# jianwang-mpi/GlobalEgoMocap

Hardware: AMD Instinct MI355X
Metric: optimised windows/sec (10-frame, 15-joint) (higher is better)
Workload: dtype f32

## Files before the change

globalegomocap_amd/csrc/energy.hip:

```cpp
#include "energy_device.h"

namespace gem {

__global__ void pack_pose_kernel(const float* __restrict__ src, float* __restrict__ dst, int rows, int C) {
    const int i = blockIdx.x * blockDim.x + threadIdx.x;
    if (i >= rows * PAD) return;
    const int r = i / PAD, c = i % PAD;
    dst[i] = c < C ? src[(size_t)r * C + c] : 0.f;
}
__global__ void unpack_pose_kernel(const float* __restrict__ src, float* __restrict__ dst, int rows, int C) {
    const int i = blockIdx.x * blockDim.x + threadIdx.x;
    if (i >= rows * C) return;
    const int r = i / C, c = i % C;
    dst[i] = src[(size_t)r * PAD + c];
}
int launch_pack_pose(const float* src, float* dst, int rows, int C, hipStream_t s) {
    const int n = rows * PAD;
    hipLaunchKernelGGL(pack_pose_kernel, dim3((n + 255) / 256), dim3(256), 0, s, src, dst, rows, C);
    GEM_HIP(hipGetLastError());
    return 0;
}
int launch_unpack_pose(const float* src, float* dst, int rows, int C, hipStream_t s) {
    const int n = rows * C;
    hipLaunchKernelGGL(unpack_pose_kernel, dim3((n + 255) / 256), dim3(256), 0, s, src, dst, rows, C);
// ... 78 lines not shown
    hipLaunchKernelGGL(energy_kernel, dim3(B), dim3(64), 0, s, a);
    GEM_HIP(hipGetLastError());
    if (prof) { GEM_HIP(hipEventRecord(rec.b, s)); h->prof.recs.push_back(rec); }
    commit_kernel_names(h, prof ? rec.family : -1);
    return 0;
}

__global__ __launch_bounds__(256) void mean_bone_kernel(const float* __restrict__ pose, int n_frames, int J,
                                                        const int* __restrict__ parents, float* __restrict__ out) {
    __shared__ float red[4][MAXJ];
    const int tid = threadIdx.x, lane = tid & 63, wave = tid >> 6;
    for (int j = 0; j < J; ++j) {
        float acc = 0.f;
        const int par = parents[j];
        for (int f = tid; f < n_frames; f += 256) {
            const float* a = pose + ((size_t)f * J + j) * 3;
            const float* p = pose + ((size_t)f * J + par) * 3;
            const float dx = a[0] - p[0], dy = a[1] - p[1], dz = a[2] - p[2];
            acc += sqrtf(dx * dx + dy * dy + dz * dz);
        }
#pragma unroll
        for (int o = 32; o > 0; o >>= 1) acc += __shfl_xor(acc, o, 64);
        if (lane == 0) red[wave][j] = acc;
    }
    __syncthreads();
    if (tid < J) out[tid] = (red[0][tid] + red[1][tid] + red[2][tid] + red[3][tid]) / (float)n_frames;
}
int launch_mean_bone(gem_handle* h, const float* pose, int n_frames, float* out, hipStream_t s) {
    hipLaunchKernelGGL(mean_bone_kernel, dim3(1), dim3(256), 0, s, pose, n_frames, h->J, h->d_parents, out);
    GEM_HIP(hipGetLastError());
    return 0;
}

__global__ void gather_windows_kernel(const float* __restrict__ frames, const int32_t* __restrict__ frame0,
                                      float* __restrict__ out, int B, int T, int JC) {
    const int i = blockIdx.x * blockDim.x + threadIdx.x;
    if (i >= B * T * JC) return;
    const int b = i / (T * JC), r = i - b * T * JC;
    out[i] = frames[(size_t)frame0[b] * JC + r];
}
int launch_gather_windows(const float* frames, const int32_t* frame0, float* out, int B, int T, int JC, hipStream_t s) {
    const int n = B * T * JC;
    hipLaunchKernelGGL(gather_windows_kernel, dim3((n + 255) / 256), dim3(256), 0, s, frames, frame0, out, B, T, JC);
    GEM_HIP(hipGetLastError());
    return 0;
}

__device__ void inv4_rigid_general(const double* m, double* o) {
    const double a = m[0], b = m[1], c = m[2], d = m[4], e = m[5], f = m[6], g = m[8], hh = m[9], i = m[10];
    const double A = e * i - f * hh, Bc = -(d * i - f * g), Cc = d * hh - e * g;
    const double det = a * A + b * Bc + c * Cc;
    const double id = 1.0 / det;
    double r[9] = {A * id, -(b * i - c * hh) * id, (b * f - c * e) * id,
                   Bc * id, (a * i - c * g) * id, -(a * f - c * d) * id,
                   Cc * id, -(a * hh - b * g) * id, (a * e - b * d) * id};
    const double tx = m[3], ty = m[7], tz = m[11];
    for (int q = 0; q < 3; ++q) {
        o[q * 4 + 0] = r[q * 3 + 0]; o[q * 4 + 1] = r[q * 3 + 1]; o[q * 4 + 2] = r[q * 3 + 2];
        o[q * 4 + 3] = -(r[q * 3 + 0] * tx + r[q * 3 + 1] * ty + r[q * 3 + 2] * tz);
    }
    o[12] = 0; o[13] = 0; o[14] = 0; o[15] = 1;
}

__global__ __launch_bounds__(64) void relative_global_kernel(const float* __restrict__ local, const double* __restrict__ cams,
                                                             const int32_t* __restrict__ frame0, float* __restrict__ rel,
                                                             int T, int J) {
    __shared__ double M[MAXT][12];
    const int b = blockIdx.x, lane = threadIdx.x;
    const double* c0 = cams + (size_t)frame0[b] * 16;
    if (lane < T) {
        double inv0[16];
        inv4_rigid_general(c0, inv0);
        const double* ct = c0 + (size_t)lane * 16;
        for (int r = 0; r < 3; ++r)
            for (int c = 0; c < 4; ++c) {
                double acc = 0;
                for (int k = 0; k < 4; ++k) acc += inv0[r * 4 + k] * ct[k * 4 + c];
                M[lane][r * 4 + c] = acc;
            }
    }
    __syncthreads();
    for (int p = lane; p < T * J; p += 64) {
        const int t = p / J;
        const float* x = local + ((size_t)b * T * J + p) * 3;
        const double X = x[0], Y = x[1], Z = x[2];
        float* o = rel + ((size_t)b * T * J + p) * 3;
        for (int r = 0; r < 3; ++r)
            o[r] = (float)(M[t][r * 4 + 0] * X + M[t][r * 4 + 1] * Y + M[t][r * 4 + 2] * Z + M[t][r * 4 + 3]);
    }
}
__global__ __launch_bounds__(64) void to_global_kernel(const float* __restrict__ rel, const double* __restrict__ cams,
                                                       const int32_t* __restrict__ frame0, double* __restrict__ out, int T, int J) {
    const int b = blockIdx.x, lane = threadIdx.x;
    const double* c0 = cams + (size_t)frame0[b] * 16;
    for (int p = lane; p < T * J; p += 64) {
        const float* x = rel + ((size_t)b * T * J + p) * 3;
        const double X = x[0], Y = x[1], Z = x[2];
        double* o = out + ((size_t)b * T * J + p) * 3;
        for (int r = 0; r < 3; ++r) o[r] = c0[r * 4 + 0] * X + c0[r * 4 + 1] * Y + c0[r * 4 + 2] * Z + c0[r * 4 + 3];
    }
}
int launch_relative_global(const float* local, const double* cams, const int32_t* frame0, float* rel, int B, int T, int J,
                           hipStream_t s) {
    hipLaunchKernelGGL(relative_global_kernel, dim3(B), dim3(64), 0, s, local, cams, frame0, rel, T, J);
    GEM_HIP(hipGetLastError());
    return 0;
}
int launch_to_global(const float* rel, const double* cams, const int32_t* frame0, double* out, int B, int T, int J,
                     hipStream_t s) {
    hipLaunchKernelGGL(to_global_kernel, dim3(B), dim3(64), 0, s, rel, cams, frame0, out, T, J);
    GEM_HIP(hipGetLastError());
    return 0;
}

}
```

globalegomocap_amd/csrc/gem_api.hip:

```cpp
#include <cxxabi.h>

#include <algorithm>
#include <cmath>
#include <cstdio>
#include <cstdlib>
#include <cstring>
#include <memory>

#include "gem_internal.h"

namespace gem {

static thread_local std::string g_error;
void set_error(const std::string& msg) { g_error = msg; }
bool hip_ok(hipError_t e, const char* what) {
    if (e == hipSuccess) return true;
    g_error = std::string(what) + ": " + hipGetErrorString(e);
    return false;
}

const char* dev_env(const char* name) {
    const char* on = getenv("GEM_DEV");
    if (!on || on[0] != '1') return nullptr;
    return getenv(name);
}

void note_kernel(gem_handle* h, const void* host_fn) {
    if (!h->prof.on) return;
    const char* m = hipKernelNameRefByPtr(host_fn, nullptr);
    if (!m) return;
    int st = 0;
    char* d = abi::__cxa_demangle(m, nullptr, nullptr, &st);
    std::string n = (st == 0 && d) ? d : m;
    free(d);
    if (n.rfind("void ", 0) == 0) n = n.substr(5);
    int depth = 0;
    for (size_t i = 0; i < n.size(); ++i) {
        if (n[i] == '<') ++depth;
        else if (n[i] == '>') --depth;
        else if (n[i] == '(' && depth == 0) { n.resize(i); break; }
    }
    h->prof.pending.insert(n);
}

static void drop_graphs(gem_handle* h) {
    for (auto& g : h->graphs) { if (g.exec) (void)hipGraphExecDestroy(g.exec); if (g.graph) (void)hipGraphDestroy(g.graph); }
    h->graphs.clear();
}

__global__ void fill_u32_kernel(uint32_t* __restrict__ p, uint32_t v, size_t n) {
    const size_t i = (size_t)blockIdx.x * blockDim.x + threadIdx.x;
    if (i < n) p[i] = v;
}
static int launch_fill_u32(uint32_t* p, uint32_t v, size_t n, hipStream_t s) {
    if (!n) return 0;
    hipLaunchKernelGGL(fill_u32_kernel, dim3((unsigned)((n + 255) / 256)), dim3(256), 0, s, p, v, n);
    GEM_HIP(hipGetLastError());
    return 0;
}

template <typename T>
static int dev_alloc(std::vector<void*>& owner, T** p, size_t n) {
    void* q = nullptr;
    GEM_HIP(hipMalloc(&q, (n ? n : 1) * sizeof(T)));
    owner.push_back(q);
    *p = static_cast<T*>(q);
    GEM_HIP(hipMemset(q, 0, (n ? n : 1) * sizeof(T)));
    return 0;
}
static void free_all(std::vector<void*>& owner) {
    for (void* p : owner) (void)hipFree(p);
    owner.clear();
}

template <typename T>
static int upload(std::vector<void*>& owner, T** p, const std::vector<T>& v) {
    if (dev_alloc(owner, p, v.size())) return 1;
    GEM_HIP(hipMemcpy(*p, v.data(), v.size() * sizeof(T), hipMemcpyHostToDevice));
    return 0;
}

static uint16_t host_f2bf(float x) {
    uint32_t u;
    std::memcpy(&u, &x, 4);
    return (uint16_t)((u + 0x7FFFu + ((u >> 16) & 1u)) >> 16);
}
static float host_bf2f(uint16_t b) {
    const uint32_t u = (uint32_t)b << 16;
    float f;
    std::memcpy(&f, &u, 4);
    return f;
// ... 331 lines not shown
        net.dec_bwd.push_back(Lb);
        return 0;
    };
    for (int i = nh - 1; i >= 1; --i)
        if (add_dec(c.hidden[i], c.hidden[i - 1], true, true)) return 1;
    if (add_dec(c.hidden[0], c.hidden[0], true, true)) return 1;
    if (add_dec(c.hidden[0], C, false, false)) return 1;
    net.tail_start = -1;
    if (!dev_env("GEM_NO_TAIL"))
        for (int st = 1; st < (int)net.dec.size(); ++st) {
            const size_t bytes = plan_tail(net.dec, st, T, h->J, nullptr);
            if (bytes && bytes <= 160 * 1024) { net.tail_start = st; net.tail_lds = bytes; break; }
        }
    if (net.tail_start == 1 && !dev_env("GEM_NO_FRONT") && compose_front(h, net, first_conv, dec_in_bias_tm.data())) return 1;
    if (build_tail_bf16_stream(h, net)) return 1;
    net.host_fwd.clear(); net.host_fwd.shrink_to_fit();
    net.host_bwd.clear(); net.host_bwd.shrink_to_fit();
    net.loaded = true;
    return 0;
}

}

namespace gem {

static int check_call(gem_handle* h, int stage, int B, const char* who) {
    if (!h) { set_error(std::string(who) + ": null handle"); return 1; }
    if (stage < 0 || stage > 1 || !h->net[stage].loaded) { set_error(std::string(who) + ": VAE weights of this stage are not loaded"); return 1; }
    if (B < 0 || B > h->ws.Bmax) { set_error(std::string(who) + ": B exceeds max_windows"); return 1; }
    GEM_HIP(hipSetDevice(h->cfg.device));
    return 0;
}

static int encoder_forward(gem_handle* h, int stage, int B, const float* d_pose, hipStream_t s) {
    StageNet& net = h->net[stage];
    Workspace& w = h->ws;
    const int rows = B * h->T;
    if (launch_pack_pose(d_pose, w.pose_p, rows, h->C, s)) return 1;
    const float* in = w.pose_p;
    int lda = PAD;
    for (size_t i = 0; i < net.enc.size(); ++i) {
        if (launch_gemm(h, net.enc[i], EPI_BIAS_LRELU, in, lda, nullptr, w.enc_act[i], net.enc[i].N, rows, h->T, s, -1)) return 1;
        in = w.enc_act[i];
        lda = net.enc[i].N;
    }
    return launch_gemm(h, net.fc, EPI_BIAS, in, net.fc.K, nullptr, w.mulv, net.fc.N, B, h->T, s, -1);
}

static int decoder_forward(gem_handle* h, int stage, int B, const float* zp, hipStream_t s) {
    StageNet& net = h->net[stage];
    Workspace& w = h->ws;
    const int rows = B * h->T;
    const bool front = net.front.w && net.dec.size() > 1 && h->precision != GEM_PRECISION_BF16;
    const float* in = w.h0;
    if (front) {
        if (launch_gemm(h, net.front, EPI_BIAS_LRELU, zp, h->Dp, nullptr, w.dec_act[0], net.front.N, B, h->T, s, 0, w.dyn ? w.perm : nullptr)) return 1;
        in = w.dec_act[0];
    } else if (launch_gemm(h, net.dec_in, EPI_BIAS, zp, h->Dp, nullptr, w.h0, net.dec_in.N, B, h->T, s, 0, w.dyn ? w.perm : nullptr)) {
        return 1;
    }
    for (size_t i = front ? 1 : 0; i < net.dec.size(); ++i) {
        const int epi = (i + 1 < net.dec.size()) ? EPI_BIAS_LRELU : EPI_BIAS;
        if (launch_gemm(h, net.dec[i], epi, in, net.dec[i].K, nullptr, w.dec_act[i], net.dec[i].N, rows, h->T, s, -1)) return 1;
        in = w.dec_act[i];
    }
    return 0;
}

static int decoder_backward(gem_handle* h, int stage, int B, hipStream_t s, int from, const float* gin) {
    StageNet& net = h->net[stage];
    Workspace& w = h->ws;
// ... 74 lines not shown
    ta.B = B; ta.forward_only = forward_only ? 1 : 0; ta.dbg_ts = nullptr;
    ta.in_slab = in_slab; ta.in_bias = front ? net.front.bias : net.dec[st - 1].bias;
    ta.in_bias_ld = front ? net.dec[0].N : 0;
    for (int i = 0; i < ta.n; ++i) {
        const Layer& f = net.dec[st + i];
        const Layer& g = net.dec_bwd[st + i];
        ta.fwd[i] = TailLayerDev{f.w4, f.bias, f.K, f.N};
        ta.bwd[i] = TailLayerDev{g.w4, nullptr, g.K, g.N};
    }
    ta.a_in = w.dec_act[st - 1]; ta.g_out = w.dec_grad[st]; ta.g_out_b = nullptr; ta.Xp = (w.dyn && !forward_only) ? nullptr : w.dec_act.back();
    ta.e = ea;
    if (launch_tail(h, ta, tail_lds, s)) return 1;
    if (forward_only) return 0;
    if (front) {
        w.defer_reduce = w.dyn;
        const int rc = launch_gemm(h, net.front_bwd, EPI_BIAS, w.dec_grad[st], net.front_bwd.K, nullptr, w.dz, h->Dp, B, h->T, s, 0);
        w.grad_slab = w.defer_reduce ? w.deferred : SlabSrc{};
        w.defer_reduce = false;
        return rc;
    }
    return decoder_backward(h, stage, B, s, st - 1, w.dec_grad[st]);
}

struct StageRun {
    gem_handle* h = nullptr;
    int stage = 0, B = 0;
    const float* pose_in = nullptr; const float* heat = nullptr; const int32_t* frame0 = nullptr; const float* mean_bone = nullptr;
    const float* eps = nullptr;
    gem_energy_weights wt{}; gem_lbfgs_opts opt{};
    float* pose_out = nullptr; gem_window_stats* stats = nullptr;
    hipStream_t s = nullptr;
    EnergyArgs ea{};
    bool fuse = false;
    bool atomic_slots = false;
    long log0 = 0;
    int rounds = 0;
};

static void compaction_home(Workspace& w) {
    w.perm = w.perm_home; w.slot_of = w.slot_of_home; w.n_active = w.n_active_home;
    w.next_perm = w.next_slot_of = w.next_count = nullptr;
}

static int stage_begin(StageRun& r) {
    gem_handle* h = r.h;
    Workspace& w = h->ws;
    const int B = r.B, stage = r.stage;
    hipStream_t s = r.s;
    if (r.wt.reproj != 0.0 && (!r.heat || !r.frame0)) { set_error("optimize: reproj weight != 0 needs heat-maps and frame indices"); return 1; }
    if (r.opt.max_iter < 1 || r.opt.max_eval < 1 || r.opt.max_iter - 1 > w.hist_cap || r.opt.max_iter > MAX_HIST) {
        set_error("optimize: max_iter must be 1.." + std::to_string(w.hist_cap + 1)); return 1;
    }
    if (r.opt.max_eval > 1021) { set_error("optimize: max_eval must be at most 1021 (torch's default for max_iter = 25 is 31)"); return 1; }
    r.rounds = r.opt.max_eval + 1;
    if (B == 0) return 0;
    if (encoder_forward(h, stage, B, r.pose_in, s)) return 1;
    if (launch_reparam(w.mulv, r.eps, nullptr, nullptr, nullptr, w.trial, B, h->D, h->Dp, s)) return 1;
    if (h->precision == GEM_PRECISION_BF16 && launch_f32_to_bf16(w.trial, w.trial_b, (size_t)B * h->Dp, s)) return 1;
    if (launch_lbfgs_init(h, B, r.opt, s)) return 1;
    compaction_home(w);
    StageNet& net_ = h->net[stage];
    const bool front_ = net_.front.w && net_.tail_start == 1 && h->precision != GEM_PRECISION_BF16;
    const Layer& first_ = front_ ? net_.front : net_.dec_in;
    const int tail_g_ = h->T <= 16 ? 16 / h->T : 1;
    const bool tail_path_ = net_.tail_start >= 0 && (B + tail_g_ - 1) / tail_g_ <= tail_cap_workgroups(h, net_.dec, net_.tail_start);
    const bool fuse_ = tail_path_ && rows_can_fuse_compaction(h, first_, h->Dp, first_.N, B, front_);
    r.atomic_slots = bf16_rounds_take_slots_atomically(h, stage, B) ||
                     (h->precision == GEM_PRECISION_F32 && front_ && tail_path_ && !fuse_);
    if (r.atomic_slots) {
        if ((w.log_pos % N_LOG) + r.rounds + 2 > N_LOG) w.log_pos += N_LOG - (w.log_pos % N_LOG);
        r.log0 = w.log_pos;
    }
    if (launch_compact(h, B, 1, s, r.atomic_slots ? r.rounds + 1 : 0)) return 1;
    if (r.atomic_slots) w.log_pos = r.log0 + r.rounds + 2;
    w.dyn = true;
    w.tex_on = h->tex_cache && w.tex_key && r.wt.reproj != 0.0;
    if (w.tex_on && launch_fill_u32(reinterpret_cast<uint32_t*>(w.tex_key), 0xFFFFFFFFu, (size_t)B * h->T * h->J, s)) return 1;
    r.ea = energy_args(h, r.pose_in, r.heat, r.frame0, r.mean_bone, r.wt);
    w.tex_on = false;
    if (launch_fill_u32(reinterpret_cast<uint32_t*>(w.trace), 0xFFFFFFFFu, (size_t)TRACE_ROUNDS * w.Bmax * 2, s)) return 1;
    r.fuse = fuse_;
    return 0;
}

static int stage_round(StageRun& r, int k) {
    gem_handle* h = r.h;
    Workspace& w = h->ws;
    if (r.B == 0) return 0;
    int rc = 0;
    w.round = k;
    if (r.atomic_slots) {
        int* cnt = w.n_log + (r.log0 + k) % N_LOG;
        w.perm = (k & 1) ? w.perm2 : w.perm_home;       w.next_perm = (k & 1) ? w.perm_home : w.perm2;
        w.slot_of = (k & 1) ? w.slot_of2 : w.slot_of_home; w.next_slot_of = (k & 1) ? w.slot_of_home : w.slot_of2;
        w.n_active = cnt; w.next_count = cnt + 1;
        w.cur_log = r.log0 + k;
        r.ea.n_dev = w.n_active; r.ea.perm = w.perm;
    } else
    if (k > 0) {
        if (r.fuse) {
            w.fuse_compact = true;
            w.fuse_log = w.n_log + (w.log_pos % N_LOG);
            w.cur_log = w.log_pos++;
        } else {
            rc = launch_compact(h, r.B, 0, r.s);
        }
    }
    rc = rc || evaluate(h, r.stage, r.B, w.trial, r.ea, r.s);
    if (!rc) rc = launch_lbfgs_advance(h, r.B, r.opt, r.s);
    if (w.fuse_compact) { set_error("optimize: the fused compaction was not picked up"); rc = 1; w.fuse_compact = false; }
    w.round = -1;
    return rc;
}

static int stage_finish(StageRun& r) {
    gem_handle* h = r.h;
    Workspace& w = h->ws;
    w.round = -1;
    w.dyn = false;
    compaction_home(w);
    if (r.B == 0) return 0;
    if (evaluate(h, r.stage, r.B, w.trial, energy_args(h, r.pose_in, r.heat, r.frame0, r.mean_bone, r.wt), r.s, true)) return 1;
    if (launch_unpack_pose(w.dec_act.back(), r.pose_out, r.B * h->T, h->C, r.s)) return 1;
    if (r.stats && launch_lbfgs_stats(h, r.B, r.stats, r.s)) return 1;
    return 0;
}

static int optimize_stage_impl(gem_handle* h, int stage, int B, const float* d_pose_in, const float* d_heat,
                               const int32_t* d_frame0, const float* d_mean_bone, const float* d_eps,
                               const gem_energy_weights& wt, const gem_lbfgs_opts& opt, float* d_pose_out,
                               gem_window_stats* d_stats, hipStream_t s) {
    StageRun r;
    r.h = h; r.stage = stage; r.B = B; r.pose_in = d_pose_in; r.heat = d_heat; r.frame0 = d_frame0; r.mean_bone = d_mean_bone; r.eps = d_eps;
    r.wt = wt; r.opt = opt; r.pose_out = d_pose_out; r.stats = d_stats; r.s = s;
    if (stage_begin(r)) { h->ws.dyn = false; compaction_home(h->ws); return 1; }
    int rc = 0;
    for (int k = 0; k < r.rounds && !rc; ++k) rc = stage_round(r, k);
    if (rc) { h->ws.round = -1; h->ws.dyn = false; compaction_home(h->ws); return 1; }
    return stage_finish(r);
}

struct WindowsRun {
    gem_handle* h = nullptr;
    int B = 0;
    const float* local_pose = nullptr; const double* cams = nullptr; const float* heat = nullptr; const int32_t* frame0 = nullptr;
    const float* mean_bone = nullptr; const float* eps_local = nullptr; const float* eps_global = nullptr;
    gem_energy_weights w_local{}, w_global{}; gem_lbfgs_opts opt{};
    float* mid_local = nullptr; double* global = nullptr; gem_window_stats* stats_local = nullptr; gem_window_stats* stats_global = nullptr;
    hipStream_t s = nullptr;
    StageRun st;
    float* mid = nullptr;
};

static int windows_begin_local(WindowsRun& r) {
    gem_handle* h = r.h;
    Workspace& w = h->ws;
    if (launch_gather_windows(r.local_pose, r.frame0, w.pose_a, r.B, h->T, h->C, r.s)) return 1;
    r.mid = r.mid_local ? r.mid_local : w.pose_b;
    StageRun& s = r.st;
    s = StageRun{};
    s.h = h; s.stage = GEM_STAGE_LOCAL; s.B = r.B; s.pose_in = w.pose_a; s.heat = r.heat; s.frame0 = r.frame0; s.mean_bone = r.mean_bone;
    s.eps = r.eps_local; s.wt = r.w_local; s.opt = r.opt; s.pose_out = r.mid; s.stats = r.stats_local; s.s = r.s;
    return stage_begin(s);
}
static int windows_begin_global(WindowsRun& r) {
    gem_handle* h = r.h;
    Workspace& w = h->ws;
    if (stage_finish(r.st)) return 1;
    if (launch_relative_global(r.mid, r.cams, r.frame0, w.pose_a, r.B, h->T, h->J, r.s)) return 1;
    StageRun& s = r.st;
    s = StageRun{};
    s.h = h; s.stage = GEM_STAGE_GLOBAL; s.B = r.B; s.pose_in = w.pose_a; s.heat = r.heat; s.frame0 = r.frame0; s.mean_bone = r.mean_bone;
    s.eps = r.eps_global; s.wt = r.w_global; s.opt = r.opt; s.pose_out = w.pose_b;
    s.stats = r.stats_global; s.s = r.s;
    return stage_begin(s);
}
static int windows_end(WindowsRun& r) {
    gem_handle* h = r.h;
    if (stage_finish(r.st)) return 1;
    return launch_to_global(h->ws.pose_b, r.cams, r.frame0, r.global, r.B, h->T, h->J, r.s);
}
static void windows_abort(WindowsRun& r) { r.h->ws.round = -1; r.h->ws.dyn = false; compaction_home(r.h->ws); }

static int windows_single(WindowsRun& r) {
    int rc = windows_begin_local(r);
    for (int k = 0; k < r.st.rounds && !rc; ++k) rc = stage_round(r.st, k);
    rc = rc || windows_begin_global(r);
    for (int k = 0; k < r.st.rounds && !rc; ++k) rc = stage_round(r.st, k);
    rc = rc || windows_end(r);
    if (rc) windows_abort(r);
    return rc;
}

static bool same_key(const GraphKey& a, const GraphKey& b) {
    if (a.kind != b.kind || a.stage != b.stage || a.B != b.B || a.precision != b.precision || a.stream != b.stream || a.tex_cache != b.tex_cache)
        return false;
    for (int i = 0; i < 12; ++i)
        if (a.ptr[i] != b.ptr[i]) return false;
    return std::memcmp(a.w, b.w, sizeof(a.w)) == 0 && std::memcmp(&a.opt, &b.opt, sizeof(a.opt)) == 0;
}

template <typename Body>
static int run_graphed(gem_handle* h, const GraphKey& key, hipStream_t s, Body body) {
    if (!h->graphs_on || s == nullptr || h->prof.on) return body();
    GraphEntry* e = nullptr;
    for (auto& g : h->graphs)
        if (same_key(g.key, key)) { e = &g; break; }
    ++h->graph_tick;
    if (!e) {
        if (h->graphs.size() >= 16) {
            size_t lru = 0;
            for (size_t i = 1; i < h->graphs.size(); ++i)
                if (h->graphs[i].last_use < h->graphs[lru].last_use) lru = i;
// ... 294 lines not shown
```

globalegomocap_amd/csrc/gem_internal.h:

```cpp
#pragma once
#if defined(__HIP_DEVICE_COMPILE__) && !defined(GEM_NO_PACKED_FP32)
#error "compile with: -Xclang -target-feature -Xclang -packed-fp32-ops -DGEM_NO_PACKED_FP32 (__graft_entry__.NO_PACKED_FP32)"
#endif

#include <hip/hip_runtime.h>
#include <stdint.h>
#include <atomic>
#include <set>
#include <string>
#include <vector>

#include "../../include/gem_hip.h"

namespace gem {

constexpr int PAD = 64;
constexpr float LEAKY_SLOPE = 0.01f;
constexpr double BN_EPS = 1e-5;
constexpr int MAX_HIST = 128;
constexpr int MAXJ_ERR = GEM_MAX_JOINTS;
constexpr int N_LOG = 1 << 16;
constexpr int TRACE_ROUNDS = 64;

inline int pad64(int x) { return (x + PAD - 1) / PAD * PAD; }
// ... 181 lines not shown
    int64_t graph_replays = 0, graph_captures = 0;
    int* d_parents = nullptr;
    int* d_children = nullptr;
};

namespace gem {

void note_kernel(gem_handle* h, const void* host_fn);
inline void commit_kernel_names(gem_handle* h, int family) {
    if (family >= 0 && family < 4) h->prof.names[family].insert(h->prof.pending.begin(), h->prof.pending.end());
    h->prof.pending.clear();
}

int launch_gemm(gem_handle* h, const Layer& L, int epi, const float* A, int lda, const float* aux, float* Cout, int ldc,
                int M, int T, hipStream_t s, int family, const int* row_map = nullptr);

int pick_splitk(const gem_handle* h, long blocks, int n_tiles, size_t slab_elems);

struct DynSplit { int RT, SK, per; size_t slab; };
__host__ __device__ inline DynSplit dyn_split(int M, int BM, int CT, int W, int n_tiles, int ldc) {
    DynSplit d;
    d.RT = (M + BM - 1) / BM;
    if (d.RT < 1) d.RT = 1;
    int cap = W / (d.RT * CT);
    if (cap < 1) cap = 1;
    int mx = n_tiles / 4;
    if (mx < 1) mx = 1;
    const int sk = cap < mx ? cap : mx;
    d.per = (n_tiles + sk - 1) / sk;
    d.SK = (n_tiles + d.per - 1) / d.per;
    d.slab = (size_t)d.RT * BM * ldc;
    return d;
}
__device__ inline void slab_layout(const SlabSrc& s, int& nslab, size_t& stride) {
    nslab = s.nslab;
    stride = s.stride;
    if (s.dyn_W > 0) {
        const DynSplit d = dyn_split(*s.m_dev, 64, s.CT, s.dyn_W, s.n_tiles, s.ldc);
        nslab = d.SK;
        stride = d.slab;
    }
}
bool rows_can_fuse_compaction(const gem_handle* h, const Layer& L, int lda, int ldc, int B, bool slabs);
bool bf16_rounds_take_slots_atomically(const gem_handle* h, int stage, int B);
int launch_splitk_reduce(gem_handle* h, int epi, int nslab, size_t slab, const float* bias, const float* aux, float* C, int M, int N,
                         int ldc, const int* m_dev, hipStream_t s, int dyn_W = 0, int n_tiles = 0);
int launch_gemm_bf16(gem_handle* h, const Layer& L, int epi, int nprod, const float* A, int lda, const float* aux, float* Cout,
                     int ldc, int M, int T, hipStream_t s, const int* row_map);

struct EnergyArgs;
int evaluate_bf16(gem_handle* h, int stage, int B, const EnergyArgs& ea, hipStream_t s, bool forward_only);
int launch_f32_to_bf16(const float* src, uint16_t* dst, size_t n, hipStream_t s);
int launch_f32_split_bf16(const float* src, uint16_t* hi, uint16_t* lo, size_t n, hipStream_t s);

int launch_pack_pose(const float* src, float* dst, int rows, int C, hipStream_t s);
int launch_unpack_pose(const float* src, float* dst, int rows, int C, hipStream_t s);
int launch_reparam(const float* mulv, const float* eps, float* mu, float* logvar, float* z, float* z2, int B, int D, int Dp,
                   hipStream_t s);
int launch_pad_latent(const float* z, float* zp, int B, int D, int Dp, hipStream_t s);
int launch_unpad_latent(const float* zp, float* z, int B, int D, int Dp, hipStream_t s);

struct EnergyArgs {
    const float* Xp;
    const float* X0;
    const float* heat;
    const int32_t* frame0;
// ... 33 lines not shown
    int off_act[TAIL_MAX_LAYERS + 1], ld_act[TAIL_MAX_LAYERS + 1], off_g[2], ld_g, off_red, off_escr, off_zero, off_pre;
    EnergyArgs e;
};
size_t plan_tail(const std::vector<Layer>& dec, int start, int T, int J, TailArgs* out, bool shared = false);
size_t plan_tail_for(const gem_handle* h, const std::vector<Layer>& dec, int start, int wgs, TailArgs* out);

constexpr int TB_MAX_LAYERS = 6;
struct TailB16Layer { int K, N; const float* bias; };
struct TailB16Args {
    int n, B, G, nrt, forward_only, mask_first;
    SlabSrc in_slab;
    const float* in_bias;
    int in_bias_ld;
    const uint16_t* a_in_b;
    uint16_t* g_out_b;
    float* Xp;
    long long* dbg_ts;
    const uint16_t* wstream;
    int steps_f, steps_total;
    TailB16Layer fwd[TB_MAX_LAYERS], bwd[TB_MAX_LAYERS];
    int off_act[TB_MAX_LAYERS + 1], ld_act[TB_MAX_LAYERS + 1];
    int off_mask[TB_MAX_LAYERS], ld_mask[TB_MAX_LAYERS];
    int off_x, escr, off_mb, off_zero, off_tab;
    int off_bwin, off_epair;
    EnergyArgs e;
};
size_t plan_tail_bf16(const std::vector<Layer>& dec, int start, int T, int J, TailB16Args* out, int nrt = 5);
int tail_bf16_row_tiles(const gem_handle* h, int B, int T);
int build_tail_bf16_stream(gem_handle* h, StageNet& net);
int launch_tail_bf16(gem_handle* h, const TailB16Args& a, size_t lds_bytes, hipStream_t s);
int launch_tail(gem_handle* h, const TailArgs& a, size_t lds_bytes, hipStream_t s);
int tail_cap_workgroups(const gem_handle* h, const std::vector<Layer>& dec, int start);
int launch_mean_bone(gem_handle* h, const float* pose, int n_frames, float* out, hipStream_t s);
int launch_gather_windows(const float* frames, const int32_t* frame0, float* out, int B, int T, int JC, hipStream_t s);
int launch_relative_global(const float* local, const double* cams, const int32_t* frame0, float* rel, int B, int T, int J,
                           hipStream_t s);
int launch_to_global(const float* rel, const double* cams, const int32_t* frame0, double* out, int B, int T, int J,
                     hipStream_t s);

int launch_errors(gem_handle* h, const double* est, const double* mid, const double* opt, const double* gt, int F,
                  const double* bone_mm, double* frame_out, double* out, hipStream_t s, int n_seq);
int launch_merge(const double* win, double* tmp, double* out, int n_chunks, int wpc, int T, int JC, int overlap, int smooth,
                 hipStream_t s);
size_t errors_frame_lds_bytes(int J);
int post_scratch(gem_handle* h, size_t elems);
int launch_lift(gem_handle* h, const float* heat, const double* depth, int F, const double* poly, int n_poly, int up, int pad_x,
                int pad_y, double* out64, float* out32, hipStream_t s);

int launch_lbfgs_init(gem_handle* h, int B, const gem_lbfgs_opts& o, hipStream_t s);
int launch_lbfgs_advance(gem_handle* h, int B, const gem_lbfgs_opts& o, hipStream_t s);
int launch_lbfgs_stats(gem_handle* h, int B, gem_window_stats* out, hipStream_t s);
int launch_compact(gem_handle* h, int B, int force_all, hipStream_t s, int zero_after = 0);


}
```

globalegomocap_amd/csrc/lbfgs.hip:

```cpp
#include "gem_internal.h"

namespace gem {

typedef float f32x4 __attribute__((ext_vector_type(4)));

enum { PH_INIT = 0, PH_BRACKET = 1, PH_ZOOM = 2, PH_DONE = 3 };
static_assert(PH_DONE == 3, "Workspace::done_phase (gem_internal.h) names this value for the fused compaction of gemm_rows.h");

struct AdvArgs {
    LbfgsState* state;
    const double* f;
    double* trace;
    const float* gnew;
    float *x, *d, *g, *gp, *bg0, *bg1, *trial, *S, *Y;
    uint16_t* trial_b;
    int* phase_arr;
    const int* slot_of;
    int *next_perm, *next_slot_of, *next_count;
    SlabSrc gslab;
    unsigned long long* clk;
    int Dp, hist_cap;
    gem_lbfgs_opts o;
};

__device__ __forceinline__ double cubic_interpolate(double x1, double f1, double g1, double x2, double f2, double g2,
                                                    bool has_bounds, double lo, double hi) {
    if (!has_bounds) {
        lo = x1 <= x2 ? x1 : x2;
        hi = x1 <= x2 ? x2 : x1;
    }
    const double d1 = g1 + g2 - 3.0 * (f1 - f2) / (x1 - x2);
    const double d2s = d1 * d1 - g1 * g2;
// ... 531 lines not shown
    if (tid == 0) {
        if (a.next_count && phase != PH_DONE) {
            const int slot = atomicAdd(a.next_count, 1);
            a.next_perm[slot] = b;
            a.next_slot_of[b] = slot;
        }
        if (a.phase_arr) a.phase_arr[b] = phase;
        sp->phase = phase; sp->n_iter = n_iter; sp->evals = evals; sp->ls_iter = ls_iter; sp->ls_evals = ls_evals;
        sp->max_ls = max_ls; sp->first_bracket = first_bracket; sp->ls_done = ls_done; sp->insuf = insuf;
        sp->low = low; sp->high = high; sp->hist_count = hist_count; sp->hist_start = hist_start;
        sp->loss = loss; sp->prev_loss = prev_loss; sp->t = t; sp->gtd = gtd; sp->d_norm = d_norm; sp->H_diag = H_diag;
        sp->t_prev = t_prev; sp->f_prev = f_prev; sp->gtd_prev = gtd_prev;
        sp->br_t[0] = br_t[0]; sp->br_t[1] = br_t[1]; sp->br_f[0] = br_f[0]; sp->br_f[1] = br_f[1];
        sp->br_gtd[0] = br_gtd[0]; sp->br_gtd[1] = br_gtd[1];
    }
    LB_PROBE(9);
#ifdef GEM_LB_PROBE
    if (a.clk && tid == 0 && full_path) {
        unsigned long long prev = ts[0];
#pragma unroll
        for (int i = 1; i < 10; ++i)
            if (ts[i]) { atomicAdd(a.clk + i, ts[i] - prev); prev = ts[i]; }
        atomicAdd(a.clk + 30, (unsigned long long)hist_count);
        atomicAdd(a.clk + 31, 1ull);
    }
#endif
    (void)full_path;
#undef LB_PROBE
}

template <int EPT, bool FULL, bool HB = false>
__global__ __launch_bounds__(256) void lbfgs_advance_kernel(AdvArgs a) { lbfgs_advance_body<EPT, 256, FULL, HB>(a); }

__global__ void lbfgs_init_kernel(LbfgsState* st, int* __restrict__ phase_arr, const float* __restrict__ trial, float* __restrict__ x, int B,
                                  int Dp) {
    const size_t i = (size_t)blockIdx.x * blockDim.x + threadIdx.x;
    if (i < (size_t)B * Dp) x[i] = trial[i];
    if (i < (size_t)B) {
        phase_arr[i] = PH_INIT;
        LbfgsState* s = st + i;
        s->phase = PH_INIT; s->n_iter = 0; s->evals = 0; s->ls_iter = 0; s->ls_evals = 0; s->max_ls = 0;
        s->first_bracket = 0; s->ls_done = 0; s->insuf = 0; s->low = 0; s->high = 1; s->hist_count = 0; s->hist_start = 0;
        s->nan_seen = 0;
        s->loss = 0; s->prev_loss = 0; s->t = 0; s->gtd = 0; s->d_norm = 0; s->H_diag = 1;
        s->t_prev = 0; s->f_prev = 0; s->gtd_prev = 0;
        s->br_t[0] = s->br_t[1] = 0; s->br_f[0] = s->br_f[1] = 0; s->br_gtd[0] = s->br_gtd[1] = 0;
    }
}

__global__ void lbfgs_stats_kernel(const LbfgsState* st, gem_window_stats* out, int B) {
    const int i = blockIdx.x * blockDim.x + threadIdx.x;
    if (i >= B) return;
    out[i].n_iter = st[i].n_iter;
    out[i].func_evals = st[i].evals;
    out[i].final_loss = (float)st[i].loss;
    out[i].status = (st[i].phase == PH_DONE ? 1 : 0) | (st[i].nan_seen ? 2 : 0);
}

static AdvArgs make_args(gem_handle* h, const gem_lbfgs_opts& o) {
    Workspace& w = h->ws;
    AdvArgs a;
    a.state = w.state; a.f = w.f; a.gnew = w.dz;
    a.trace = (w.round >= 0 && w.round < TRACE_ROUNDS) ? w.trace + (size_t)w.round * w.Bmax : nullptr;
    a.x = w.x; a.d = w.d; a.g = w.g; a.gp = w.gp; a.bg0 = w.bg0; a.bg1 = w.bg1; a.trial = w.trial; a.S = w.S; a.Y = w.Y;
    a.trial_b = h->precision == GEM_PRECISION_BF16 ? w.trial_b : nullptr;
    a.phase_arr = w.phase;
    a.slot_of = w.dyn ? w.slot_of : nullptr;
    a.next_perm = w.dyn ? w.next_perm : nullptr; a.next_slot_of = w.dyn ? w.next_slot_of : nullptr; a.next_count = w.dyn ? w.next_count : nullptr;
    a.gslab = w.dyn ? w.grad_slab : SlabSrc{};
    a.clk = w.lbfgs_clk;
    a.Dp = h->Dp; a.hist_cap = w.hist_cap; a.o = o;
    return a;
}

int launch_lbfgs_init(gem_handle* h, int B, const gem_lbfgs_opts& o, hipStream_t s) {
    (void)o;
    const size_t n = (size_t)B * h->Dp;
    hipLaunchKernelGGL(lbfgs_init_kernel, dim3((unsigned)((n + 255) / 256)), dim3(256), 0, s, h->ws.state, h->ws.phase, h->ws.trial, h->ws.x,
                       B, h->Dp);
    GEM_HIP(hipGetLastError());
    return 0;
}

int launch_lbfgs_advance(gem_handle* h, int B, const gem_lbfgs_opts& o, hipStream_t s) {
    AdvArgs a = make_args(h, o);
    Profile::Rec rec;
    const bool prof = h->prof.on;
    if (prof) {
        GEM_HIP(hipEventCreate(&rec.a)); GEM_HIP(hipEventCreate(&rec.b));
        rec.family = 2; rec.flops = 0;
        GEM_HIP(hipEventRecord(rec.a, s));
    }
    const int ept = (h->Dp + 255) / 256;
    typedef void (*kern_t)(AdvArgs);
    kern_t kern = nullptr;
    if (ept <= 1) kern = lbfgs_advance_kernel<1, false>;
    else if (ept <= 2) kern = lbfgs_advance_kernel<2, false>;
    else if (ept <= 4) kern = lbfgs_advance_kernel<4, false>;
    else if (h->Dp == 2048 && h->precision == GEM_PRECISION_BF16) kern = lbfgs_advance_kernel<8, true, true>;
    else if (h->Dp == 2048) kern = lbfgs_advance_kernel<8, true>;
    else if (ept <= 8) kern = lbfgs_advance_kernel<8, false>;
    else if (ept <= 16) kern = lbfgs_advance_kernel<16, false>;
    else { set_error("latent_dim > 4096 is not supported by the L-BFGS kernel"); return 1; }
    note_kernel(h, reinterpret_cast<const void*>(kern));
    hipLaunchKernelGGL(kern, dim3(B), dim3(256), 0, s, a);
    GEM_HIP(hipGetLastError());
    if (prof) { GEM_HIP(hipEventRecord(rec.b, s)); h->prof.recs.push_back(rec); }
    commit_kernel_names(h, prof ? 2 : -1);
    return 0;
}

__global__ __launch_bounds__(1024) void compact_kernel(const int* __restrict__ phase_arr, int B, int T, int* __restrict__ perm,
                                                       int* __restrict__ slot_of, int* __restrict__ n_active, int force_all,
// ... 11 lines not shown
#pragma unroll
    for (int d = 1; d < 64; d <<= 1) {
        const int v = __shfl_up(incl, d);
        if (lane >= d) incl += v;
    }
    if (lane == 63) wsum[wave] = incl;
    __syncthreads();
    int woff = 0, total = 0;
#pragma unroll
    for (int i = 0; i < 16; ++i) { if (i < wave) woff += wsum[i]; total += wsum[i]; }
    int pa = woff + incl - cnt;
    int pi = total + (b0 - pa);
    for (int e = 0; e < E; ++e) {
        const int b = b0 + e;
        if (b >= B) break;
        if ((mask >> e) & 1ull) { perm[pa] = b; slot_of[b] = pa++; }
        else { perm[pi] = b; slot_of[b] = pi++; }
    }
    if (tid == 0) { n_active[0] = total; n_active[1] = total * T; *log_slot = total; }
    if (tid < zero_after) log_slot[1 + tid] = 0;
}

int launch_compact(gem_handle* h, int B, int force_all, hipStream_t s, int zero_after) {
    Workspace& w = h->ws;
    if (B > 65536) { set_error("compact: more than 65536 windows per call"); return 1; }
    if (zero_after < 0 || zero_after > 1024 || (w.log_pos % N_LOG) + zero_after >= N_LOG) { set_error("compact: bad counter range"); return 1; }
    hipLaunchKernelGGL(compact_kernel, dim3(1), dim3(1024), 0, s, w.phase, B, h->T, w.perm, w.slot_of, w.n_active, force_all,
                       w.n_log + (w.log_pos % N_LOG), zero_after);
    GEM_HIP(hipGetLastError());
    w.cur_log = w.log_pos++;
    return 0;
}

int launch_lbfgs_stats(gem_handle* h, int B, gem_window_stats* out, hipStream_t s) {
    hipLaunchKernelGGL(lbfgs_stats_kernel, dim3((B + 255) / 256), dim3(256), 0, s, h->ws.state, out, B);
    GEM_HIP(hipGetLastError());
    return 0;
}

}
```

Before: 32080.

## Fuse stage setup and teardown kernels into single open and close launches

Several small per-stage kernels are merged. Reparameterisation, L-BFGS init, compaction reset and the trace and texture-key fills now run in one stage_open kernel. Unpack, stats and the to-global transform now run in one stage_close kernel. The window gather and relative-global transforms also write the padded encoder input directly, so the separate pack kernel is skipped. The goal is to cut kernel launch count and redundant passes over global memory on a latency-bound small workload. The cost is larger, more coupled kernels, and references to new fields such as done_phase, whose definitions cannot be confirmed from the code shown.

Measured after the change: 32210 (median of 6 runs). Within noise of the previous version (+0.4%).

```diff
diff --git a/globalegomocap_amd/csrc/energy.hip b/globalegomocap_amd/csrc/energy.hip
--- a/globalegomocap_amd/csrc/energy.hip
+++ b/globalegomocap_amd/csrc/energy.hip
@@ -134,16 +134,22 @@
     return 0;
 }
 
-__global__ void gather_windows_kernel(const float* __restrict__ frames, const int32_t* __restrict__ frame0,
-                                      float* __restrict__ out, int B, int T, int JC) {
-    const int i = blockIdx.x * blockDim.x + threadIdx.x;
-    if (i >= B * T * JC) return;
-    const int b = i / (T * JC), r = i - b * T * JC;
-    out[i] = frames[(size_t)frame0[b] * JC + r];
-}
-int launch_gather_windows(const float* frames, const int32_t* frame0, float* out, int B, int T, int JC, hipStream_t s) {
-    const int n = B * T * JC;
-    hipLaunchKernelGGL(gather_windows_kernel, dim3((n + 255) / 256), dim3(256), 0, s, frames, frame0, out, B, T, JC);
+__global__ void gather_windows_packed_kernel(const float* __restrict__ frames, const int32_t* __restrict__ frame0, float* __restrict__ out,
+                                             float* __restrict__ packed, int B, int T, int JC) {
+    const int i = blockIdx.x * blockDim.x + threadIdx.x;
+    if (i >= B * T * PAD) return;
+    const int row = i / PAD, c = i % PAD, b = row / T, t = row - b * T;
+    float v = 0.f;
+    if (c < JC) {
+        v = frames[(size_t)frame0[b] * JC + t * JC + c];
+        out[(size_t)row * JC + c] = v;
+    }
+    packed[i] = v;
+}
+int launch_gather_windows_packed(const float* frames, const int32_t* frame0, float* out, float* packed, int B, int T, int JC, hipStream_t s) {
+    if (JC > PAD) { set_error("gather_windows: more than 64 pose values per frame"); return 1; }
+    const int n = B * T * PAD;
+    hipLaunchKernelGGL(gather_windows_packed_kernel, dim3((n + 255) / 256), dim3(256), 0, s, frames, frame0, out, packed, B, T, JC);
     GEM_HIP(hipGetLastError());
     return 0;
 }
@@ -166,7 +172,7 @@
 
 __global__ __launch_bounds__(64) void relative_global_kernel(const float* __restrict__ local, const double* __restrict__ cams,
                                                              const int32_t* __restrict__ frame0, float* __restrict__ rel,
-                                                             int T, int J) {
+                                                             float* __restrict__ packed, int T, int J) {
     __shared__ double M[MAXT][12];
     const int b = blockIdx.x, lane = threadIdx.x;
     const double* c0 = cams + (size_t)frame0[b] * 16;
@@ -187,32 +193,54 @@
         const float* x = local + ((size_t)b * T * J + p) * 3;
         const double X = x[0], Y = x[1], Z = x[2];
         float* o = rel + ((size_t)b * T * J + p) * 3;
-        for (int r = 0; r < 3; ++r)
+        float* q = packed ? packed + ((size_t)b * T + t) * PAD + (p - t * J) * 3 : nullptr;
+        for (int r = 0; r < 3; ++r) {
             o[r] = (float)(M[t][r * 4 + 0] * X + M[t][r * 4 + 1] * Y + M[t][r * 4 + 2] * Z + M[t][r * 4 + 3]);
-    }
-}
-__global__ __launch_bounds__(64) void to_global_kernel(const float* __restrict__ rel, const double* __restrict__ cams,
-                                                       const int32_t* __restrict__ frame0, double* __restrict__ out, int T, int J) {
-    const int b = blockIdx.x, lane = threadIdx.x;
-    const double* c0 = cams + (size_t)frame0[b] * 16;
-    for (int p = lane; p < T * J; p += 64) {
-        const float* x = rel + ((size_t)b * T * J + p) * 3;
-        const double X = x[0], Y = x[1], Z = x[2];
-        double* o = out + ((size_t)b * T * J + p) * 3;
-        for (int r = 0; r < 3; ++r) o[r] = c0[r * 4 + 0] * X + c0[r * 4 + 1] * Y + c0[r * 4 + 2] * Z + c0[r * 4 + 3];
-    }
-}
-int launch_relative_global(const float* local, const double* cams, const int32_t* frame0, float* rel, int B, int T, int J,
-                           hipStream_t s) {
-    hipLaunchKernelGGL(relative_global_kernel, dim3(B), dim3(64), 0, s, local, cams, frame0, rel, T, J);
-    GEM_HIP(hipGetLastError());
-    return 0;
-}
-int launch_to_global(const float* rel, const double* cams, const int32_t* frame0, double* out, int B, int T, int J,
-                     hipStream_t s) {
-    hipLaunchKernelGGL(to_global_kernel, dim3(B), dim3(64), 0, s, rel, cams, frame0, out, T, J);
-    GEM_HIP(hipGetLastError());
-    return 0;
-}
-
-}
+            if (q) q[r] = o[r];
+        }
+    }
+    if (packed) {
+        const int C = J * 3, padc = PAD - C;
+        for (int e = lane; e < T * padc; e += 64) packed[((size_t)b * T + e / padc) * PAD + C + e % padc] = 0.f;
+    }
+}
+__device__ __forceinline__ void to_global_point(const double* __restrict__ c0, const float* __restrict__ x, double* __restrict__ o) {
+    const double X = x[0], Y = x[1], Z = x[2];
+    for (int r = 0; r < 3; ++r) o[r] = c0[r * 4 + 0] * X + c0[r * 4 + 1] * Y + c0[r * 4 + 2] * Z + c0[r * 4 + 3];
+}
+__global__ __launch_bounds__(64) void stage_close_kernel(const float* __restrict__ padded, float* __restrict__ pose_out,
+                                                         const LbfgsState* __restrict__ st, gem_window_stats* __restrict__ stats,
+                                                         int done_phase, const double* __restrict__ cams,
+                                                         const int32_t* __restrict__ frame0, double* __restrict__ glob, int T, int J) {
+    const int b = blockIdx.x, lane = threadIdx.x, C = J * 3;
+    const float* src = padded + (size_t)b * T * PAD;
+    for (int e = lane; e < T * C; e += 64) pose_out[(size_t)b * T * C + e] = src[(e / C) * PAD + e % C];
+    if (stats && lane == 0) {
+        stats[b].n_iter = st[b].n_iter;
+        stats[b].func_evals = st[b].evals;
+        stats[b].final_loss = (float)st[b].loss;
+        stats[b].status = (st[b].phase == done_phase ? 1 : 0) | (st[b].nan_seen ? 2 : 0);
+    }
+    if (glob) {
+        const double* c0 = cams + (size_t)frame0[b] * 16;
+        for (int p = lane; p < T * J; p += 64) {
+            const int t = p / J;
+            to_global_point(c0, src + t * PAD + (p - t * J) * 3, glob + ((size_t)b * T * J + p) * 3);
+        }
+    }
+}
+int launch_stage_close(gem_handle* h, const float* padded, float* pose_out, gem_window_stats* stats, const double* cams,
+                       const int32_t* frame0, double* glob, int B, hipStream_t s) {
+    hipLaunchKernelGGL(stage_close_kernel, dim3(B), dim3(64), 0, s, padded, pose_out, h->ws.state, stats, h->ws.done_phase, cams, frame0,
+                       glob, h->T, h->J);
+    GEM_HIP(hipGetLastError());
+    return 0;
+}
+int launch_relative_global_packed(const float* local, const double* cams, const int32_t* frame0, float* rel, float* packed, int B, int T,
+                                  int J, hipStream_t s) {
+    hipLaunchKernelGGL(relative_global_kernel, dim3(B), dim3(64), 0, s, local, cams, frame0, rel, packed, T, J);
+    GEM_HIP(hipGetLastError());
+    return 0;
+}
+
+}
diff --git a/globalegomocap_amd/csrc/gem_api.hip b/globalegomocap_amd/csrc/gem_api.hip
--- a/globalegomocap_amd/csrc/gem_api.hip
+++ b/globalegomocap_amd/csrc/gem_api.hip
@@ -46,17 +46,6 @@
 static void drop_graphs(gem_handle* h) {
     for (auto& g : h->graphs) { if (g.exec) (void)hipGraphExecDestroy(g.exec); if (g.graph) (void)hipGraphDestroy(g.graph); }
     h->graphs.clear();
-}
-
-__global__ void fill_u32_kernel(uint32_t* __restrict__ p, uint32_t v, size_t n) {
-    const size_t i = (size_t)blockIdx.x * blockDim.x + threadIdx.x;
-    if (i < n) p[i] = v;
-}
-static int launch_fill_u32(uint32_t* p, uint32_t v, size_t n, hipStream_t s) {
-    if (!n) return 0;
-    hipLaunchKernelGGL(fill_u32_kernel, dim3((unsigned)((n + 255) / 256)), dim3(256), 0, s, p, v, n);
-    GEM_HIP(hipGetLastError());
-    return 0;
 }
 
 template <typename T>
@@ -454,11 +443,11 @@
     return 0;
 }
 
-static int encoder_forward(gem_handle* h, int stage, int B, const float* d_pose, hipStream_t s) {
+static int encoder_forward(gem_handle* h, int stage, int B, const float* d_pose, hipStream_t s, bool packed = false) {
     StageNet& net = h->net[stage];
     Workspace& w = h->ws;
     const int rows = B * h->T;
-    if (launch_pack_pose(d_pose, w.pose_p, rows, h->C, s)) return 1;
+    if (!packed && launch_pack_pose(d_pose, w.pose_p, rows, h->C, s)) return 1;
     const float* in = w.pose_p;
     int lda = PAD;
     for (size_t i = 0; i < net.enc.size(); ++i) {
@@ -599,6 +588,8 @@
     hipStream_t s = nullptr;
     EnergyArgs ea{};
     bool fuse = false;
+    bool packed_in = false;
+    const double* cams = nullptr; double* glob = nullptr;
     bool atomic_slots = false;
     long log0 = 0;
     int rounds = 0;
@@ -621,10 +612,7 @@
     if (r.opt.max_eval > 1021) { set_error("optimize: max_eval must be at most 1021 (torch's default for max_iter = 25 is 31)"); return 1; }
     r.rounds = r.opt.max_eval + 1;
     if (B == 0) return 0;
-    if (encoder_forward(h, stage, B, r.pose_in, s)) return 1;
-    if (launch_reparam(w.mulv, r.eps, nullptr, nullptr, nullptr, w.trial, B, h->D, h->Dp, s)) return 1;
-    if (h->precision == GEM_PRECISION_BF16 && launch_f32_to_bf16(w.trial, w.trial_b, (size_t)B * h->Dp, s)) return 1;
-    if (launch_lbfgs_init(h, B, r.opt, s)) return 1;
+    if (encoder_forward(h, stage, B, r.pose_in, s, r.packed_in)) return 1;
     compaction_home(w);
     StageNet& net_ = h->net[stage];
     const bool front_ = net_.front.w && net_.tail_start == 1 && h->precision != GEM_PRECISION_BF16;
@@ -638,14 +626,13 @@
         if ((w.log_pos % N_LOG) + r.rounds + 2 > N_LOG) w.log_pos += N_LOG - (w.log_pos % N_LOG);
         r.log0 = w.log_pos;
     }
-    if (launch_compact(h, B, 1, s, r.atomic_slots ? r.rounds + 1 : 0)) return 1;
+    w.tex_on = h->tex_cache && w.tex_key && r.wt.reproj != 0.0;
+    if (launch_stage_open(h, B, r.eps, r.atomic_slots ? r.rounds + 1 : 0, w.tex_on ? (size_t)B * h->T * h->J : 0, s)) return 1;
+    if (h->precision == GEM_PRECISION_BF16 && launch_f32_to_bf16(w.trial, w.trial_b, (size_t)B * h->Dp, s)) return 1;
     if (r.atomic_slots) w.log_pos = r.log0 + r.rounds + 2;
     w.dyn = true;
-    w.tex_on = h->tex_cache && w.tex_key && r.wt.reproj != 0.0;
-    if (w.tex_on && launch_fill_u32(reinterpret_cast<uint32_t*>(w.tex_key), 0xFFFFFFFFu, (size_t)B * h->T * h->J, s)) return 1;
     r.ea = energy_args(h, r.pose_in, r.heat, r.frame0, r.mean_bone, r.wt);
     w.tex_on = false;
-    if (launch_fill_u32(reinterpret_cast<uint32_t*>(w.trace), 0xFFFFFFFFu, (size_t)TRACE_ROUNDS * w.Bmax * 2, s)) return 1;
     r.fuse = fuse_;
     return 0;
 }
@@ -688,9 +675,7 @@
     compaction_home(w);
     if (r.B == 0) return 0;
     if (evaluate(h, r.stage, r.B, w.trial, energy_args(h, r.pose_in, r.heat, r.frame0, r.mean_bone, r.wt), r.s, true)) return 1;
-    if (launch_unpack_pose(w.dec_act.back(), r.pose_out, r.B * h->T, h->C, r.s)) return 1;
-    if (r.stats && launch_lbfgs_stats(h, r.B, r.stats, r.s)) return 1;
-    return 0;
+    return launch_stage_close(h, w.dec_act.back(), r.pose_out, r.stats, r.cams, r.frame0, r.glob, r.B, r.s);
 }
 
 static int optimize_stage_impl(gem_handle* h, int stage, int B, const float* d_pose_in, const float* d_heat,
@@ -722,30 +707,31 @@
 static int windows_begin_local(WindowsRun& r) {
     gem_handle* h = r.h;
     Workspace& w = h->ws;
-    if (launch_gather_windows(r.local_pose, r.frame0, w.pose_a, r.B, h->T, h->C, r.s)) return 1;
+    if (launch_gather_windows_packed(r.local_pose, r.frame0, w.pose_a, w.pose_p, r.B, h->T, h->C, r.s)) return 1;
     r.mid = r.mid_local ? r.mid_local : w.pose_b;
     StageRun& s = r.st;
     s = StageRun{};
     s.h = h; s.stage = GEM_STAGE_LOCAL; s.B = r.B; s.pose_in = w.pose_a; s.heat = r.heat; s.frame0 = r.frame0; s.mean_bone = r.mean_bone;
     s.eps = r.eps_local; s.wt = r.w_local; s.opt = r.opt; s.pose_out = r.mid; s.stats = r.stats_local; s.s = r.s;
+    s.packed_in = true;
     return stage_begin(s);
 }
 static int windows_begin_global(WindowsRun& r) {
     gem_handle* h = r.h;
     Workspace& w = h->ws;
     if (stage_finish(r.st)) return 1;
-    if (launch_relative_global(r.mid, r.cams, r.frame0, w.pose_a, r.B, h->T, h->J, r.s)) return 1;
+    if (launch_relative_global_packed(r.mid, r.cams, r.frame0, w.pose_a, w.pose_p, r.B, h->T, h->J, r.s)) return 1;
     StageRun& s = r.st;
     s = StageRun{};
     s.h = h; s.stage = GEM_STAGE_GLOBAL; s.B = r.B; s.pose_in = w.pose_a; s.heat = r.heat; s.frame0 = r.frame0; s.mean_bone = r.mean_bone;
     s.eps = r.eps_global; s.wt = r.w_global; s.opt = r.opt; s.pose_out = w.pose_b;
     s.stats = r.stats_global; s.s = r.s;
+    s.packed_in = true;
+    s.cams = r.cams; s.glob = r.global;
     return stage_begin(s);
 }
 static int windows_end(WindowsRun& r) {
-    gem_handle* h = r.h;
-    if (stage_finish(r.st)) return 1;
-    return launch_to_global(h->ws.pose_b, r.cams, r.frame0, r.global, r.B, h->T, h->J, r.s);
+    return stage_finish(r.st);
 }
 static void windows_abort(WindowsRun& r) { r.h->ws.round = -1; r.h->ws.dyn = false; compaction_home(r.h->ws); }
 
diff --git a/globalegomocap_amd/csrc/gem_internal.h b/globalegomocap_amd/csrc/gem_internal.h
--- a/globalegomocap_amd/csrc/gem_internal.h
+++ b/globalegomocap_amd/csrc/gem_internal.h
@@ -237,6 +237,12 @@
     d.slab = (size_t)d.RT * BM * ldc;
     return d;
 }
+__device__ __forceinline__ float reparam_value(const float* __restrict__ mulv, const float* __restrict__ eps, int b, int k, int D, int Dp) {
+    if (k >= D) return 0.f;
+    const float m = mulv[(size_t)b * 2 * Dp + k];
+    const float lv = mulv[(size_t)b * 2 * Dp + Dp + k];
+    return eps ? eps[(size_t)b * D + k] * expf(0.5f * lv) + m : m;
+}
 __device__ inline void slab_layout(const SlabSrc& s, int& nslab, size_t& stride) {
     nslab = s.nslab;
     stride = s.stride;
@@ -336,11 +342,11 @@
 int launch_tail(gem_handle* h, const TailArgs& a, size_t lds_bytes, hipStream_t s);
 int tail_cap_workgroups(const gem_handle* h, const std::vector<Layer>& dec, int start);
 int launch_mean_bone(gem_handle* h, const float* pose, int n_frames, float* out, hipStream_t s);
-int launch_gather_windows(const float* frames, const int32_t* frame0, float* out, int B, int T, int JC, hipStream_t s);
-int launch_relative_global(const float* local, const double* cams, const int32_t* frame0, float* rel, int B, int T, int J,
-                           hipStream_t s);
-int launch_to_global(const float* rel, const double* cams, const int32_t* frame0, double* out, int B, int T, int J,
-                     hipStream_t s);
+int launch_gather_windows_packed(const float* frames, const int32_t* frame0, float* out, float* packed, int B, int T, int JC, hipStream_t s);
+int launch_relative_global_packed(const float* local, const double* cams, const int32_t* frame0, float* rel, float* packed, int B, int T,
+                                  int J, hipStream_t s);
+int launch_stage_close(gem_handle* h, const float* padded, float* pose_out, gem_window_stats* stats, const double* cams,
+                       const int32_t* frame0, double* glob, int B, hipStream_t s);
 
 int launch_errors(gem_handle* h, const double* est, const double* mid, const double* opt, const double* gt, int F,
                   const double* bone_mm, double* frame_out, double* out, hipStream_t s, int n_seq);
@@ -351,9 +357,8 @@
 int launch_lift(gem_handle* h, const float* heat, const double* depth, int F, const double* poly, int n_poly, int up, int pad_x,
                 int pad_y, double* out64, float* out32, hipStream_t s);
 
-int launch_lbfgs_init(gem_handle* h, int B, const gem_lbfgs_opts& o, hipStream_t s);
+int launch_stage_open(gem_handle* h, int B, const float* eps, int zero_after, size_t tex_n, hipStream_t s);
 int launch_lbfgs_advance(gem_handle* h, int B, const gem_lbfgs_opts& o, hipStream_t s);
-int launch_lbfgs_stats(gem_handle* h, int B, gem_window_stats* out, hipStream_t s);
 int launch_compact(gem_handle* h, int B, int force_all, hipStream_t s, int zero_after = 0);
 
 
diff --git a/globalegomocap_amd/csrc/lbfgs.hip b/globalegomocap_amd/csrc/lbfgs.hip
--- a/globalegomocap_amd/csrc/lbfgs.hip
+++ b/globalegomocap_amd/csrc/lbfgs.hip
@@ -1,3 +1,5 @@
+#include <algorithm>
+
 #include "gem_internal.h"
 
 namespace gem {
@@ -595,10 +597,18 @@
 template <int EPT, bool FULL, bool HB = false>
 __global__ __launch_bounds__(256) void lbfgs_advance_kernel(AdvArgs a) { lbfgs_advance_body<EPT, 256, FULL, HB>(a); }
 
-__global__ void lbfgs_init_kernel(LbfgsState* st, int* __restrict__ phase_arr, const float* __restrict__ trial, float* __restrict__ x, int B,
-                                  int Dp) {
+__global__ __launch_bounds__(256) void stage_open_kernel(LbfgsState* st, int* __restrict__ phase_arr, const float* __restrict__ mulv,
+                                                         const float* __restrict__ eps, float* __restrict__ trial, float* __restrict__ x,
+                                                         int B, int D, int Dp, int T, int* __restrict__ perm, int* __restrict__ slot_of,
+                                                         int* __restrict__ n_active, int* __restrict__ log_slot, int zero_after,
+                                                         uint32_t* __restrict__ trace, size_t n_trace, uint32_t* __restrict__ tex,
+                                                         size_t n_tex) {
     const size_t i = (size_t)blockIdx.x * blockDim.x + threadIdx.x;
-    if (i < (size_t)B * Dp) x[i] = trial[i];
+    if (i < (size_t)B * Dp) {
+        const float zz = reparam_value(mulv, eps, (int)(i / Dp), (int)(i % Dp), D, Dp);
+        trial[i] = zz;
+        x[i] = zz;
+    }
     if (i < (size_t)B) {
         phase_arr[i] = PH_INIT;
         LbfgsState* s = st + i;
@@ -608,16 +618,13 @@
         s->loss = 0; s->prev_loss = 0; s->t = 0; s->gtd = 0; s->d_norm = 0; s->H_diag = 1;
         s->t_prev = 0; s->f_prev = 0; s->gtd_prev = 0;
         s->br_t[0] = s->br_t[1] = 0; s->br_f[0] = s->br_f[1] = 0; s->br_gtd[0] = s->br_gtd[1] = 0;
-    }
-}
-
-__global__ void lbfgs_stats_kernel(const LbfgsState* st, gem_window_stats* out, int B) {
-    const int i = blockIdx.x * blockDim.x + threadIdx.x;
-    if (i >= B) return;
-    out[i].n_iter = st[i].n_iter;
-    out[i].func_evals = st[i].evals;
-    out[i].final_loss = (float)st[i].loss;
-    out[i].status = (st[i].phase == PH_DONE ? 1 : 0) | (st[i].nan_seen ? 2 : 0);
+        perm[i] = (int)i;
+        slot_of[i] = (int)i;
+    }
+    if (i == 0) { n_active[0] = B; n_active[1] = B * T; *log_slot = B; }
+    if (i < (size_t)zero_after) log_slot[1 + i] = 0;
+    if (i < n_trace) trace[i] = 0xFFFFFFFFu;
+    if (i < n_tex) tex[i] = 0xFFFFFFFFu;
 }
 
 static AdvArgs make_args(gem_handle* h, const gem_lbfgs_opts& o) {
@@ -636,12 +643,17 @@
     return a;
 }
 
-int launch_lbfgs_init(gem_handle* h, int B, const gem_lbfgs_opts& o, hipStream_t s) {
-    (void)o;
-    const size_t n = (size_t)B * h->Dp;
-    hipLaunchKernelGGL(lbfgs_init_kernel, dim3((unsigned)((n + 255) / 256)), dim3(256), 0, s, h->ws.state, h->ws.phase, h->ws.trial, h->ws.x,
-                       B, h->Dp);
+int launch_stage_open(gem_handle* h, int B, const float* eps, int zero_after, size_t tex_n, hipStream_t s) {
+    Workspace& w = h->ws;
+    if (B > 65536) { set_error("compact: more than 65536 windows per call"); return 1; }
+    if (zero_after < 0 || zero_after > 1024 || (w.log_pos % N_LOG) + zero_after >= N_LOG) { set_error("compact: bad counter range"); return 1; }
+    const size_t n_trace = (size_t)TRACE_ROUNDS * w.Bmax * 2;
+    const size_t n = std::max(std::max((size_t)B * h->Dp, n_trace), std::max(tex_n, (size_t)zero_after));
+    hipLaunchKernelGGL(stage_open_kernel, dim3((unsigned)((n + 255) / 256)), dim3(256), 0, s, w.state, w.phase, w.mulv, eps, w.trial, w.x, B,
+                       h->D, h->Dp, h->T, w.perm, w.slot_of, w.n_active, w.n_log + (w.log_pos % N_LOG), zero_after,
+                       reinterpret_cast<uint32_t*>(w.trace), n_trace, reinterpret_cast<uint32_t*>(w.tex_key), tex_n);
     GEM_HIP(hipGetLastError());
+    w.cur_log = w.log_pos++;
     return 0;
 }
 
@@ -719,10 +731,4 @@
     return 0;
 }
 
-int launch_lbfgs_stats(gem_handle* h, int B, gem_window_stats* out, hipStream_t s) {
-    hipLaunchKernelGGL(lbfgs_stats_kernel, dim3((B + 255) / 256), dim3(256), 0, s, h->ws.state, out, B);
-    GEM_HIP(hipGetLastError());
-    return 0;
-}
-
-}
+}
```
